# rowanz/merlot

Measured on NVIDIA H100. Metric: frame-caption segments/sec (fwd+bwd+AdamW), higher is better.
Workload: dtype bf16

## Files before the change

merlot_b200/csrc/attention.cu:

```cuda
#include "host_common.h"
#include "ptx.cuh"

namespace mb {

constexpr int AT_M = 128;
constexpr int AT_N = 128;
constexpr int AT_D = 64;
constexpr float LOG2E = 1.4426950408889634f;
constexpr float LN2 = 0.6931471805599453f;

struct AttnDev {
  int B, S, heads, H;
  const uint8_t* valid;
  float scale;
  bf16* ctx; int ld_ctx;
  float* lse;
  float* dsum;
  float* dq_accum; int ld_dq;
  size_t dq_part_stride;
  bf16* dqkv; int ld_dqkv;
  float* colsum;
  float* colsum2;
  int colsum_split;
  int colsum_valid_q;
// ... 140 lines not shown
    mbar_wait(&bar_kv[j & 1], (uint32_t)((j >> 1) & 1));
    const uint32_t ka = smem_u32(sKV + (j & 1) * 16384), va = ka + 8192;
    float s[32];
    wgmma_fence();
#pragma unroll
    for (int k = 0; k < AT_D / 16; ++k) wgmma_m64n64_ss<0, 0>(s, desc_kmajor(qa, k), desc_kmajor(ka, k), k > 0 ? 1u : 0u);
    wgmma_commit();
    wgmma_wait<0>();
    reg_fence(s);
    const int k0 = j * FK;
#pragma unroll
    for (int i = 0; i < 2; ++i) {
      uint32_t iw[2], vw[2];
#pragma unroll
      for (int w = 0; w < 2; ++w) {
        iw[w] = range_word(k0 + 32 * w, S);
        vw[w] = (HAS_MASK && vq[i]) ? s_mask[(k0 >> 5) + w] : 0xffffffffu;
        if (HAS_MASK && pair_lo[i] >= 0) vw[w] &= pair_word(k0 + 32 * w, pair_lo[i], p.pair_P, p.pair_chunk);
      }
      float mx = -INFINITY;
#pragma unroll
      for (int jj = 0; jj < 8; ++jj) {
#pragma unroll
        for (int e = 0; e < 2; ++e) {
          const int bit = (8 * jj + 2 * (lane & 3) + e) & 31, w = jj >> 2;
          float t = s[4 * jj + 2 * i + e] * sc2[i];
          t = ((vw[w] >> bit) & 1u) ? t : MASKED_LOG2;
          t = ((iw[w] >> bit) & 1u) ? t : -INFINITY;
          s[4 * jj + 2 * i + e] = t;
          mx = fmaxf(mx, t);
        }
      }
      quad_max(mx);
      const float m_new = fmaxf(m_run[i], mx);
      const float f = ex2_approx(m_run[i] - m_new);
      m_run[i] = m_new;
      float rs = 0.f;
#pragma unroll
      for (int jj = 0; jj < 8; ++jj) {
#pragma unroll
        for (int e = 0; e < 2; ++e) {
          const float pr = ex2_approx(s[4 * jj + 2 * i + e] - m_new);
          s[4 * jj + 2 * i + e] = pr;
          rs += pr;
          o[4 * jj + 2 * i + e] *= f;
        }
      }
      l_run[i] = l_run[i] * f + rs;
    }
    if (DROP) {
#pragma unroll
      for (int x = 0; x < 32; ++x)
        if (!((zq >> x) & 1u)) s[x] = 0.f;
    }
    wgmma_fence();
#pragma unroll
    for (int kk = 0; kk < FK / 16; ++kk) {
      uint32_t a[4];
      acc_to_afrag(s, kk, a);
      wgmma_m64n64_rs<1>(o, a, desc_mnmajor(va, kk, 0), 1u);
    }
    wgmma_commit();
    wgmma_wait<0>();
    reg_fence(o);
    __syncthreads();
    if (tid == 0 && j + 2 < n_kv) load_kv(j + 2);
  }

#pragma unroll
  for (int i = 0; i < 2; ++i) {
    quad_sum(l_run[i]);
    const int q = q0 + wg * 64 + wq * 16 + (lane >> 2) + 8 * i;
    if (!q_in[i]) continue;
    const float inv = (DROP ? p.drop_scale : 1.0f) / l_run[i];
    bf16* dst = p.ctx + (size_t)(tok0 + q) * p.ld_ctx + h * AT_D + 2 * (lane & 3);
#pragma unroll
    for (int jj = 0; jj < 8; ++jj)
      *reinterpret_cast<uint32_t*>(dst + 8 * jj) = pack_bf16x2(o[4 * jj + 2 * i] * inv, o[4 * jj + 2 * i + 1] * inv);
    if ((lane & 3) == 0 && p.lse) p.lse[((size_t)b * p.heads + h) * S + q] = (m_run[i] + log2f(l_run[i])) * LN2;
  }
}

constexpr int BQ = 64;
constexpr int MAX_DQ_PARTS = 4;
constexpr int BWD_THREADS = 256;
constexpr int BWD_SMEM = 32768 + 32768 + 16384 + 1024 + 512 + 64 + 1024;

__device__ __forceinline__ uint32_t attn_keep_bits_keyrows(const AttnDev& p, uint64_t drop_bh, uint64_t drop_key, uint64_t n16, int q0,
                                                           int lane) {
  uint32_t z = 0;
#pragma unroll
  for (int jp = 0; jp < BQ / 16; ++jp) {
#pragma unroll
    for (int e = 0; e < 2; ++e) {
      const uint64_t blk = ((drop_bh + (uint64_t)((q0 >> 4) + jp)) * 8 + 2 * (lane & 3) + e) * n16 * 8 + drop_key;
      const uint4 r = attn_dropout_words(p.drop_seed, p.drop_site, blk);
      const uint32_t w[4] = {r.x, r.y, r.z, r.w};
#pragma unroll
      for (int qh = 0; qh < 2; ++qh)
#pragma unroll
        for (int i = 0; i < 2; ++i)
          z |= ((w[2 * qh + i] >> 16) >= p.drop_thresh16 ? 1u : 0u) << (4 * (2 * jp + qh) + 2 * i + e);
    }
  }
  return z;
}

template <bool HAS_MASK, bool DQ_ATOMIC, bool DROP>
__global__ void __launch_bounds__(BWD_THREADS, 1)
attn_bwd_kernel(const __grid_constant__ CUtensorMap tm_kv, const __grid_constant__ CUtensorMap tm_q,
                const __grid_constant__ CUtensorMap tm_do, const AttnDev p) {
  extern __shared__ uint8_t smem_raw[];
  uint8_t* smem = reinterpret_cast<uint8_t*>((reinterpret_cast<uintptr_t>(smem_raw) + 1023) & ~uintptr_t(1023));
  uint8_t* sK = smem;
  uint8_t* sV = smem + 16384;
  uint8_t* sQd = smem + 32768;
  uint8_t* sdST = smem + 65536;
  float* s_nlse = reinterpret_cast<float*>(smem + 81920);
  float* s_dsum = s_nlse + 2 * BQ;
  uint32_t* s_mask = reinterpret_cast<uint32_t*>(s_dsum + 2 * BQ);
  uint64_t* bars = reinterpret_cast<uint64_t*>(reinterpret_cast<uint8_t*>(s_mask) + 512);
  uint64_t *bar_kv = bars, *bar_q = bars + 1 ;

  const int tid = threadIdx.x, lane = tid & 31;
  const int warp = __shfl_sync(0xffffffffu, tid >> 5, 0);
  const int wg = warp >> 2, wq = warp & 3;
  const int kt = blockIdx.x, h = blockIdx.y, b = blockIdx.z;
  pdl_launch_dependents();
  const int S = p.S, H = p.H;
  const int k0 = kt * AT_N, tok0 = b * S;
  const int n_q = (S + BQ - 1) / BQ;

  if (tid == 0) {
    tma_prefetch_desc(&tm_kv); tma_prefetch_desc(&tm_q); tma_prefetch_desc(&tm_do);
    mbar_init(bar_kv, 1); mbar_init(&bar_q[0], 1); mbar_init(&bar_q[1], 1);
    fence_barrier_init();
  }
  __syncthreads();
  pdl_wait();
  auto load_q = [&](int c) {
    uint8_t* buf = sQd + (c & 1) * 16384;
    mbar_arrive_expect_tx(&bar_q[c & 1], 16384);
    tma_load_2d(buf, &tm_q, &bar_q[c & 1], h * AT_D, tok0 + c * BQ);
    tma_load_2d(buf + 8192, &tm_do, &bar_q[c & 1], h * AT_D, tok0 + c * BQ);
  };
  if (tid == 0) {
    mbar_arrive_expect_tx(bar_kv, 32768);
    tma_load_2d(sK, &tm_kv, bar_kv, H + h * AT_D, tok0 + k0);
    tma_load_2d(sV, &tm_kv, bar_kv, 2 * H + h * AT_D, tok0 + k0);
    load_q(0);
    if (n_q > 1) load_q(1);
  }
  const size_t st0 = ((size_t)b * p.heads + h) * S;
  auto stage_stats = [&](int c) {
    const int q = c * BQ + tid;
    s_nlse[(c & 1) * BQ + tid] = (q < S) ? -p.lse[st0 + q] * LOG2E : 0.f;
    s_dsum[(c & 1) * BQ + tid] = (q < S) ? p.dsum[st0 + q] : 0.f;
  };
  if (tid < BQ) stage_stats(0);
  if (HAS_MASK) build_mask(s_mask, p.valid + tok0, n_q * BQ, S);
  __syncthreads();

  bool k_in[2], vk[2];
  int pair_lo[2];
#pragma unroll
  for (int i = 0; i < 2; ++i) {
    const int kk = k0 + wg * 64 + wq * 16 + (lane >> 2) + 8 * i;
    k_in[i] = kk < S;
    vk[i] = k_in[i] ? (HAS_MASK ? p.valid[tok0 + kk] != 0 : true) : false;
    pair_lo[i] = HAS_MASK ? pair_lo_of(kk, p.pair_P, p.pair_chunk) : -1;
  }
  const float sc2 = p.scale * LOG2E;
  float dv[32], dk[32];
#pragma unroll
  for (int i = 0; i < 32; ++i) { dv[i] = 0.f; dk[i] = 0.f; }
  float* dq_base = p.dq_accum + (DQ_ATOMIC ? (size_t)0 : (size_t)kt * p.dq_part_stride);
  uint64_t drop_n16 = 0, drop_bh = 0, drop_key = 0;
  if (DROP) {
    drop_n16 = (uint64_t)((S + 15) >> 4);
    drop_bh = ((uint64_t)b * p.heads + h) * drop_n16;
    drop_key = (uint64_t)((k0 + wg * 64 + wq * 16) >> 4) * 8 + (lane >> 2);
  }

  mbar_wait(bar_kv, 0);
  const uint32_t ka = smem_u32(sK) + wg * 8192, va = smem_u32(sV) + wg * 8192;
  const uint32_t dsa = smem_u32(sdST);
  for (int c = 0; c < n_q; ++c) {
    const int bb = c & 1, q0 = c * BQ;
    mbar_wait(&bar_q[bb], (uint32_t)((c >> 1) & 1));
    const uint32_t qa = smem_u32(sQd + bb * 16384), da = qa + 8192;
    float s[32], dp[32];
    wgmma_fence();
#pragma unroll
    for (int k = 0; k < AT_D / 16; ++k) wgmma_m64n64_ss<0, 0>(s, desc_kmajor(ka, k), desc_kmajor(qa, k), k > 0 ? 1u : 0u);
#pragma unroll
    for (int k = 0; k < AT_D / 16; ++k) wgmma_m64n64_ss<0, 0>(dp, desc_kmajor(va, k), desc_kmajor(da, k), k > 0 ? 1u : 0u);
    wgmma_commit();
    wgmma_wait<0>();
    reg_fence(s);
    reg_fence(dp);
    const float* nlse = s_nlse + bb * BQ;
    const float* dsm = s_dsum + bb * BQ;
    uint32_t iw[2], qw[2];
#pragma unroll
    for (int w = 0; w < 2; ++w) {
      iw[w] = range_word(q0 + 32 * w, S);
      qw[w] = HAS_MASK ? s_mask[(q0 >> 5) + w] : 0xffffffffu;
    }
    const uint32_t zk = DROP ? attn_keep_bits_keyrows(p, drop_bh, drop_key, drop_n16, q0, lane) : 0u;
#pragma unroll
    for (int i = 0; i < 2; ++i) {
      uint32_t aw[2];
#pragma unroll
      for (int w = 0; w < 2; ++w)
        aw[w] = (HAS_MASK && pair_lo[i] >= 0) ? pair_word(q0 + 32 * w, pair_lo[i], p.pair_P, p.pair_chunk) : 0xffffffffu;
      const int row = wg * 64 + wq * 16 + (lane >> 2) + 8 * i;
#pragma unroll
      for (int jj = 0; jj < 8; ++jj) {
        float pv[2], dsv[2];
#pragma unroll
        for (int e = 0; e < 2; ++e) {
          const int col = 8 * jj + 2 * (lane & 3) + e, bit = col & 31, w = jj >> 2;
          float t = s[4 * jj + 2 * i + e] * sc2;
          t = (vk[i] && ((aw[w] >> bit) & 1u)) ? t : MASKED_LOG2;
          t = ((qw[w] >> bit) & 1u) ? t : 0.f;
          float pr = ex2_approx(t + nlse[col]);
          pr = (k_in[i] && ((iw[w] >> bit) & 1u)) ? pr : 0.f;
          const float gq = ((qw[w] >> bit) & 1u) ? pr : 0.f;
          if (DROP) {
            const float zs = ((zk >> (4 * jj + 2 * i + e)) & 1u) ? p.drop_scale : 0.f;
            pv[e] = pr * zs;
            dsv[e] = (dp[4 * jj + 2 * i + e] * zs - dsm[col]) * gq;
          } else {
            pv[e] = pr;
            dsv[e] = (dp[4 * jj + 2 * i + e] - dsm[col]) * gq;
          }
        }
        s[4 * jj + 2 * i] = pv[0]; s[4 * jj + 2 * i + 1] = pv[1];
        dp[4 * jj + 2 * i] = dsv[0]; dp[4 * jj + 2 * i + 1] = dsv[1];
        *reinterpret_cast<uint32_t*>(sdST + row * 128 + ((jj ^ (row & 7)) << 4) + (lane & 3) * 4) = pack_bf16x2(dsv[0], dsv[1]);
      }
    }
    wgmma_fence();
#pragma unroll
    for (int kk = 0; kk < BQ / 16; ++kk) {
      uint32_t a[4];
      acc_to_afrag(s, kk, a);
      wgmma_m64n64_rs<1>(dv, a, desc_mnmajor(da, kk, 0), 1u);
    }
#pragma unroll
    for (int kk = 0; kk < BQ / 16; ++kk) {
      uint32_t a[4];
      acc_to_afrag(dp, kk, a);
      wgmma_m64n64_rs<1>(dk, a, desc_mnmajor(qa, kk, 0), 1u);
    }
    wgmma_commit();
    fence_proxy_async_smem();
    asm volatile("bar.sync 1, 256;" ::: "memory");
    float dq[16];
    wgmma_fence();
#pragma unroll
    for (int k = 0; k < AT_N / 16; ++k)
      wgmma_m64n32_ss<1, 1>(dq, desc_mnmajor(dsa, k, 0), desc_mnmajor(smem_u32(sK) + wg * 64, k, 0), k > 0 ? 1u : 0u);
    wgmma_commit();
    wgmma_wait<0>();
    reg_fence(dv);
    reg_fence(dk);
    reg_fence(dq);
#pragma unroll
    for (int i = 0; i < 2; ++i) {
      const int q = q0 + wq * 16 + (lane >> 2) + 8 * i;
      if (q >= S) continue;
      float* dst = dq_base + (size_t)(tok0 + q) * p.ld_dq + h * AT_D + wg * 32 + 2 * (lane & 3);
#pragma unroll
      for (int jj = 0; jj < 4; ++jj) {
        const float v0 = dq[4 * jj + 2 * i], v1 = dq[4 * jj + 2 * i + 1];
        if (DQ_ATOMIC) {
          asm volatile("red.global.add.v2.f32 [%0], {%1, %2};" ::"l"(dst + 8 * jj), "f"(v0), "f"(v1) : "memory");
        } else {
          *reinterpret_cast<float2*>(dst + 8 * jj) = make_float2(v0, v1);
        }
      }
    }
    if (tid < BQ && c + 1 < n_q) stage_stats(c + 1);
    __syncthreads();
    if (tid == 0 && c + 2 < n_q) load_q(c + 2);
  }
#pragma unroll
  for (int i = 0; i < 2; ++i) {
    const int key = k0 + wg * 64 + wq * 16 + (lane >> 2) + 8 * i;
    if (key >= S) continue;
    bf16* dst = p.dqkv + (size_t)(tok0 + key) * p.ld_dqkv + h * AT_D + 2 * (lane & 3);
#pragma unroll
    for (int jj = 0; jj < 8; ++jj) {
      *reinterpret_cast<uint32_t*>(dst + H + 8 * jj) = pack_bf16x2(dk[4 * jj + 2 * i] * p.scale, dk[4 * jj + 2 * i + 1] * p.scale);
      *reinterpret_cast<uint32_t*>(dst + 2 * H + 8 * jj) = pack_bf16x2(dv[4 * jj + 2 * i], dv[4 * jj + 2 * i + 1]);
    }
  }
}

__global__ void attn_dsum_kernel(const bf16* __restrict__ o, const bf16* __restrict__ d_o, int ld, float* __restrict__ dsum,
                                 int B, int S, int heads) {
  pdl_launch_dependents();
  pdl_wait();
  const long long gid = (long long)blockIdx.x * blockDim.x + threadIdx.x;
  const long long item = gid >> 3;
  const int sub = (int)(gid & 7);
  const long long total = (long long)B * S * heads;
  float acc = 0.f;
  if (item < total) {
    const int hh = (int)(item % heads);
    const long long tok = item / heads;
    const size_t off = (size_t)tok * ld + hh * AT_D + sub * 8;
    uint4 a = __ldg(reinterpret_cast<const uint4*>(o + off));
    uint4 g = __ldg(reinterpret_cast<const uint4*>(d_o + off));
    const uint32_t* pa = reinterpret_cast<const uint32_t*>(&a);
    const uint32_t* pg = reinterpret_cast<const uint32_t*>(&g);
#pragma unroll
    for (int i = 0; i < 4; ++i) {
      float2 x = unpack_bf16x2(pa[i]), y = unpack_bf16x2(pg[i]);
      acc += x.x * y.x + x.y * y.y;
    }
  }
  acc += __shfl_xor_sync(0xffffffffu, acc, 1);
  acc += __shfl_xor_sync(0xffffffffu, acc, 2);
  acc += __shfl_xor_sync(0xffffffffu, acc, 4);
  if (item < total && sub == 0) {
    const int hh = (int)(item % heads);
    const long long tok = item / heads;
    const int bb = (int)(tok / S), q = (int)(tok % S);
    dsum[((size_t)bb * heads + hh) * S + q] = acc;
  }
}

__global__ void __launch_bounds__(256) attn_dqkv_finish_kernel(float* __restrict__ dq, int ld_dq, bf16* __restrict__ dqkv, int ld_dqkv,
                                                               long long rows, int H, float* __restrict__ bias_grad, int n_parts,
                                                               size_t part_stride, float scale) {
  __shared__ float sred[8][256];
  pdl_launch_dependents();
  pdl_wait();
  const int lane = threadIdx.x & 31, warp = threadIdx.x >> 5;
  const int col = blockIdx.x * 256 + lane * 8;
  float acc[8] = {0, 0, 0, 0, 0, 0, 0, 0};
  if (col < 3 * H) {
    for (long long r = (long long)blockIdx.y * 8 + warp; r < rows; r += (long long)gridDim.y * 8) {
      float v[8];
      bf16* o = dqkv + (size_t)r * ld_dqkv + col;
      if (col < H) {
        float4* src = reinterpret_cast<float4*>(dq + (size_t)r * ld_dq + col);
        float4 a = src[0], b = src[1];
        if (n_parts == 0) {
          src[0] = make_float4(0.f, 0.f, 0.f, 0.f);
          src[1] = make_float4(0.f, 0.f, 0.f, 0.f);
        } else {
          for (int t = 1; t < n_parts; ++t) {
            const float4* s2 = reinterpret_cast<const float4*>(dq + (size_t)t * part_stride + (size_t)r * ld_dq + col);
            const float4 c = s2[0], d = s2[1];
            a.x += c.x; a.y += c.y; a.z += c.z; a.w += c.w;
            b.x += d.x; b.y += d.y; b.z += d.z; b.w += d.w;
          }
        }
        const uint4 pk = make_uint4(pack_bf16x2(a.x * scale, a.y * scale), pack_bf16x2(a.z * scale, a.w * scale),
                                    pack_bf16x2(b.x * scale, b.y * scale), pack_bf16x2(b.z * scale, b.w * scale));
        *reinterpret_cast<uint4*>(o) = pk;
        const uint32_t* pu = reinterpret_cast<const uint32_t*>(&pk);
#pragma unroll
        for (int i = 0; i < 4; ++i) { const float2 f = unpack_bf16x2(pu[i]); v[2 * i] = f.x; v[2 * i + 1] = f.y; }
      } else {
        const uint4 u = *reinterpret_cast<const uint4*>(o);
        const uint32_t* pu = reinterpret_cast<const uint32_t*>(&u);
#pragma unroll
        for (int i = 0; i < 4; ++i) { const float2 f = unpack_bf16x2(pu[i]); v[2 * i] = f.x; v[2 * i + 1] = f.y; }
      }
#pragma unroll
      for (int i = 0; i < 8; ++i) acc[i] += v[i];
    }
  }
#pragma unroll
  for (int i = 0; i < 8; ++i) sred[warp][lane * 8 + i] = acc[i];
  __syncthreads();
  const int c = threadIdx.x;
  if (bias_grad != nullptr && blockIdx.x * 256 + c < 3 * H) {
    float s2 = 0.f;
#pragma unroll
    for (int w = 0; w < 8; ++w) s2 += sred[w][c];
    atomicAdd(bias_grad + blockIdx.x * 256 + c, s2);
  }
}

constexpr int CS_THREADS = 256;
constexpr int CS_SMEM = 16384 + 2 * 8192 + 512 + 512 + 64 + 1024;

template <bool HAS_MASK, bool DROP>
__global__ void __launch_bounds__(CS_THREADS, 2) attn_colsum_kernel(const __grid_constant__ CUtensorMap tm_k, const __grid_constant__ CUtensorMap tm_q,
                                                                    const AttnDev p) {
  extern __shared__ uint8_t smem_raw[];
  uint8_t* smem = reinterpret_cast<uint8_t*>((reinterpret_cast<uintptr_t>(smem_raw) + 1023) & ~uintptr_t(1023));
  uint8_t* sK = smem;
  uint8_t* sQ = smem + 16384;
  float* s_nlse = reinterpret_cast<float*>(smem + 32768);
  uint32_t* s_mask = reinterpret_cast<uint32_t*>(smem + 32768 + 512);
  uint64_t* bars = reinterpret_cast<uint64_t*>(smem + 32768 + 1024);
  uint64_t *bar_k = bars, *bar_q = bars + 1 ;
  const int tid = threadIdx.x, lane = tid & 31;
  const int warp = __shfl_sync(0xffffffffu, tid >> 5, 0);
  const int wg = warp >> 2, wq = warp & 3;
  const int k0 = blockIdx.x * AT_N, h = blockIdx.y, b = blockIdx.z;
  const int S = p.S, H = p.H, tok0 = b * S;
  const int n_q = (S + BQ - 1) / BQ;
  pdl_launch_dependents();
  if (tid == 0) {
    tma_prefetch_desc(&tm_k); tma_prefetch_desc(&tm_q);
    mbar_init(bar_k, 1); mbar_init(&bar_q[0], 1); mbar_init(&bar_q[1], 1);
    fence_barrier_init();
  }
  __syncthreads();
  pdl_wait();
  auto load_q = [&](int c) {
    mbar_arrive_expect_tx(&bar_q[c & 1], 8192);
    tma_load_2d(sQ + (c & 1) * 8192, &tm_q, &bar_q[c & 1], h * AT_D, tok0 + c * BQ);
  };
  if (tid == 0) {
    mbar_arrive_expect_tx(bar_k, 16384);
    tma_load_2d(sK, &tm_k, bar_k, H + h * AT_D, tok0 + k0);
    load_q(0);
    if (n_q > 1) load_q(1);
  }
  auto stage_lse = [&](int c) {
    const int q = c * BQ + tid;
    s_nlse[(c & 1) * BQ + tid] = (q < S) ? -p.lse[((size_t)b * p.heads + h) * S + q] * LOG2E : 0.f;
  };
  if (tid < BQ) stage_lse(0);
  if (HAS_MASK) build_mask(s_mask, p.valid + tok0, n_q * BQ, S);
  __syncthreads();

  bool k_in[2], vk[2];
  int pair_lo[2];
// ... 273 lines not shown
```

merlot_b200/csrc/ptx.cuh:

```cuda
#pragma once
#include <cuda.h>
#include <cuda_runtime.h>
#include <cuda_bf16.h>
#include <stdint.h>
#include <stdio.h>

namespace mb {

typedef __nv_bfloat16 bf16;

__device__ __forceinline__ uint32_t smem_u32(const void* p) {
  return static_cast<uint32_t>(__cvta_generic_to_shared(p));
}

__device__ __forceinline__ void pdl_launch_dependents() { asm volatile("griddepcontrol.launch_dependents;" ::: "memory"); }
__device__ __forceinline__ void pdl_wait() { asm volatile("griddepcontrol.wait;" ::: "memory"); }

__device__ __forceinline__ bool elect_one() {
  uint32_t pred;
  asm volatile(
      "{\n\t.reg .pred p;\n\t"
      "elect.sync _|p, 0xffffffff;\n\t"
      "selp.u32 %0, 1, 0, p;\n\t}"
      : "=r"(pred));
  return pred != 0;
}

__device__ __forceinline__ void mbar_init(uint64_t* bar, uint32_t count) {
  asm volatile("mbarrier.init.shared::cta.b64 [%0], %1;" ::"r"(smem_u32(bar)), "r"(count) : "memory");
}
__device__ __forceinline__ void fence_barrier_init() {
  asm volatile("fence.mbarrier_init.release.cluster;" ::: "memory");
}
__device__ __forceinline__ void fence_proxy_async_smem() {
  asm volatile("fence.proxy.async.shared::cta;" ::: "memory");
}
__device__ __forceinline__ void mbar_arrive_expect_tx(uint64_t* bar, uint32_t bytes) {
  asm volatile("mbarrier.arrive.expect_tx.shared::cta.b64 _, [%0], %1;" ::"r"(smem_u32(bar)), "r"(bytes)
               : "memory");
}
__device__ __forceinline__ void mbar_arrive(uint64_t* bar) {
  asm volatile("mbarrier.arrive.shared::cta.b64 _, [%0];" ::"r"(smem_u32(bar)) : "memory");
}
__device__ __forceinline__ bool mbar_try_wait(uint64_t* bar, uint32_t parity) {
  uint32_t ok;
  asm volatile(
      "{\n\t.reg .pred p;\n\t"
      "mbarrier.try_wait.parity.shared::cta.b64 p, [%1], %2;\n\t"
      "selp.u32 %0, 1, 0, p;\n\t}"
      : "=r"(ok)
      : "r"(smem_u32(bar)), "r"(parity)
      : "memory");
  return ok != 0;
}
#ifndef MB_WAIT_LIMIT_CYCLES
#define MB_WAIT_LIMIT_CYCLES (4000000000LL)
#endif
__device__ __forceinline__ void mbar_wait(uint64_t* bar, uint32_t parity) {
  if (mbar_try_wait(bar, parity)) return;
  long long t0 = clock64();
  while (!mbar_try_wait(bar, parity)) {
    if (clock64() - t0 > MB_WAIT_LIMIT_CYCLES) asm volatile("trap;");
  }
}

__device__ __forceinline__ void mbar_wait_warp(uint64_t* bar, uint32_t parity) {
  if ((threadIdx.x & 31) == 0) mbar_wait(bar, parity);
  __syncwarp();
}

__device__ __forceinline__ void tma_prefetch_desc(const CUtensorMap* m) {
  asm volatile("prefetch.tensormap [%0];" ::"l"(reinterpret_cast<uint64_t>(m)) : "memory");
}
__device__ __forceinline__ void tma_load_2d(void* smem_dst, const CUtensorMap* m, uint64_t* bar, int c0, int c1) {
  asm volatile(
      "cp.async.bulk.tensor.2d.shared::cluster.global.mbarrier::complete_tx::bytes [%0], [%1, {%3, %4}], [%2];" ::
          "r"(smem_u32(smem_dst)),
      "l"(reinterpret_cast<uint64_t>(m)), "r"(smem_u32(bar)), "r"(c0), "r"(c1)
      : "memory");
}
__device__ __forceinline__ void tma_load_3d(void* smem_dst, const CUtensorMap* m, uint64_t* bar, int c0, int c1,
                                            int c2) {
  asm volatile(
      "cp.async.bulk.tensor.3d.shared::cluster.global.mbarrier::complete_tx::bytes [%0], [%1, {%3, %4, %5}], [%2];" ::
          "r"(smem_u32(smem_dst)),
      "l"(reinterpret_cast<uint64_t>(m)), "r"(smem_u32(bar)), "r"(c0), "r"(c1), "r"(c2)
      : "memory");
}

__device__ __forceinline__ void wgmma_fence() { asm volatile("wgmma.fence.sync.aligned;" ::: "memory"); }
__device__ __forceinline__ void wgmma_commit() { asm volatile("wgmma.commit_group.sync.aligned;" ::: "memory"); }
template <int N>
__device__ __forceinline__ void wgmma_wait() { asm volatile("wgmma.wait_group.sync.aligned %0;" ::"n"(N) : "memory"); }
template <int R>
__device__ __forceinline__ void reg_fence(float (&d)[R]) {
#pragma unroll
  for (int i = 0; i < R; ++i) asm volatile("" : "+f"(d[i])::"memory");
}

template <int TA, int TB>
__device__ __forceinline__ void wgmma_m64n32_ss(float (&d)[16], uint64_t da, uint64_t db, uint32_t scale_d) {
  asm volatile(
      "{\n\t.reg .pred p;\n\t"
      "setp.ne.b32 p, %18, 0;\n\t"
      "wgmma.mma_async.sync.aligned.m64n32k16.f32.bf16.bf16 "
      "{%0, %1, %2, %3, %4, %5, %6, %7, %8, %9, %10, %11, %12, %13, %14, %15}, %16, %17, p, 1, 1, %19, %20;\n\t}"
      : "+f"(d[0]), "+f"(d[1]), "+f"(d[2]), "+f"(d[3]), "+f"(d[4]), "+f"(d[5]), "+f"(d[6]), "+f"(d[7]), "+f"(d[8]), "+f"(d[9]), "+f"(d[10]), "+f"(d[11]), "+f"(d[12]), "+f"(d[13]), "+f"(d[14]), "+f"(d[15])
      : "l"(da), "l"(db), "r"(scale_d), "n"(TA), "n"(TB));
}
template <int TA, int TB>
__device__ __forceinline__ void wgmma_m64n64_ss(float (&d)[32], uint64_t da, uint64_t db, uint32_t scale_d) {
  asm volatile(
      "{\n\t.reg .pred p;\n\t"
      "setp.ne.b32 p, %34, 0;\n\t"
      "wgmma.mma_async.sync.aligned.m64n64k16.f32.bf16.bf16 "
      "{%0, %1, %2, %3, %4, %5, %6, %7, %8, %9, %10, %11, %12, %13, %14, %15, %16, %17, %18, %19, %20, %21, %22, %23, %24, %25, %26, %27, %28, %29, %30, %31}, %32, %33, p, 1, 1, %35, %36;\n\t}"
      : "+f"(d[0]), "+f"(d[1]), "+f"(d[2]), "+f"(d[3]), "+f"(d[4]), "+f"(d[5]), "+f"(d[6]), "+f"(d[7]), "+f"(d[8]), "+f"(d[9]), "+f"(d[10]), "+f"(d[11]), "+f"(d[12]), "+f"(d[13]), "+f"(d[14]), "+f"(d[15]), "+f"(d[16]), "+f"(d[17]), "+f"(d[18]), "+f"(d[19]), "+f"(d[20]), "+f"(d[21]), "+f"(d[22]), "+f"(d[23]), "+f"(d[24]), "+f"(d[25]), "+f"(d[26]), "+f"(d[27]), "+f"(d[28]), "+f"(d[29]), "+f"(d[30]), "+f"(d[31])
      : "l"(da), "l"(db), "r"(scale_d), "n"(TA), "n"(TB));
}
template <int TA, int TB>
__device__ __forceinline__ void wgmma_m64n128_ss(float (&d)[64], uint64_t da, uint64_t db, uint32_t scale_d) {
  asm volatile(
      "{\n\t.reg .pred p;\n\t"
      "setp.ne.b32 p, %66, 0;\n\t"
      "wgmma.mma_async.sync.aligned.m64n128k16.f32.bf16.bf16 "
      "{%0, %1, %2, %3, %4, %5, %6, %7, %8, %9, %10, %11, %12, %13, %14, %15, %16, %17, %18, %19, %20, %21, %22, %23, %24, %25, %26, %27, %28, %29, %30, %31, %32, %33, %34, %35, %36, %37, %38, %39, %40, %41, %42, %43, %44, %45, %46, %47, %48, %49, %50, %51, %52, %53, %54, %55, %56, %57, %58, %59, %60, %61, %62, %63}, %64, %65, p, 1, 1, %67, %68;\n\t}"
      : "+f"(d[0]), "+f"(d[1]), "+f"(d[2]), "+f"(d[3]), "+f"(d[4]), "+f"(d[5]), "+f"(d[6]), "+f"(d[7]), "+f"(d[8]), "+f"(d[9]), "+f"(d[10]), "+f"(d[11]), "+f"(d[12]), "+f"(d[13]), "+f"(d[14]), "+f"(d[15]), "+f"(d[16]), "+f"(d[17]), "+f"(d[18]), "+f"(d[19]), "+f"(d[20]), "+f"(d[21]), "+f"(d[22]), "+f"(d[23]), "+f"(d[24]), "+f"(d[25]), "+f"(d[26]), "+f"(d[27]), "+f"(d[28]), "+f"(d[29]), "+f"(d[30]), "+f"(d[31]), "+f"(d[32]), "+f"(d[33]), "+f"(d[34]), "+f"(d[35]), "+f"(d[36]), "+f"(d[37]), "+f"(d[38]), "+f"(d[39]), "+f"(d[40]), "+f"(d[41]), "+f"(d[42]), "+f"(d[43]), "+f"(d[44]), "+f"(d[45]), "+f"(d[46]), "+f"(d[47]), "+f"(d[48]), "+f"(d[49]), "+f"(d[50]), "+f"(d[51]), "+f"(d[52]), "+f"(d[53]), "+f"(d[54]), "+f"(d[55]), "+f"(d[56]), "+f"(d[57]), "+f"(d[58]), "+f"(d[59]), "+f"(d[60]), "+f"(d[61]), "+f"(d[62]), "+f"(d[63])
      : "l"(da), "l"(db), "r"(scale_d), "n"(TA), "n"(TB));
}
template <int TA, int TB>
__device__ __forceinline__ void wgmma_m64n192_ss(float (&d)[96], uint64_t da, uint64_t db, uint32_t scale_d) {
  asm volatile(
      "{\n\t.reg .pred p;\n\t"
      "setp.ne.b32 p, %98, 0;\n\t"
      "wgmma.mma_async.sync.aligned.m64n192k16.f32.bf16.bf16 "
      "{%0, %1, %2, %3, %4, %5, %6, %7, %8, %9, %10, %11, %12, %13, %14, %15, %16, %17, %18, %19, %20, %21, %22, %23, %24, %25, %26, %27, %28, %29, %30, %31, %32, %33, %34, %35, %36, %37, %38, %39, %40, %41, %42, %43, %44, %45, %46, %47, %48, %49, %50, %51, %52, %53, %54, %55, %56, %57, %58, %59, %60, %61, %62, %63, %64, %65, %66, %67, %68, %69, %70, %71, %72, %73, %74, %75, %76, %77, %78, %79, %80, %81, %82, %83, %84, %85, %86, %87, %88, %89, %90, %91, %92, %93, %94, %95}, %96, %97, p, 1, 1, %99, %100;\n\t}"
      : "+f"(d[0]), "+f"(d[1]), "+f"(d[2]), "+f"(d[3]), "+f"(d[4]), "+f"(d[5]), "+f"(d[6]), "+f"(d[7]), "+f"(d[8]), "+f"(d[9]), "+f"(d[10]), "+f"(d[11]), "+f"(d[12]), "+f"(d[13]), "+f"(d[14]), "+f"(d[15]), "+f"(d[16]), "+f"(d[17]), "+f"(d[18]), "+f"(d[19]), "+f"(d[20]), "+f"(d[21]), "+f"(d[22]), "+f"(d[23]), "+f"(d[24]), "+f"(d[25]), "+f"(d[26]), "+f"(d[27]), "+f"(d[28]), "+f"(d[29]), "+f"(d[30]), "+f"(d[31]), "+f"(d[32]), "+f"(d[33]), "+f"(d[34]), "+f"(d[35]), "+f"(d[36]), "+f"(d[37]), "+f"(d[38]), "+f"(d[39]), "+f"(d[40]), "+f"(d[41]), "+f"(d[42]), "+f"(d[43]), "+f"(d[44]), "+f"(d[45]), "+f"(d[46]), "+f"(d[47]), "+f"(d[48]), "+f"(d[49]), "+f"(d[50]), "+f"(d[51]), "+f"(d[52]), "+f"(d[53]), "+f"(d[54]), "+f"(d[55]), "+f"(d[56]), "+f"(d[57]), "+f"(d[58]), "+f"(d[59]), "+f"(d[60]), "+f"(d[61]), "+f"(d[62]), "+f"(d[63]), "+f"(d[64]), "+f"(d[65]), "+f"(d[66]), "+f"(d[67]), "+f"(d[68]), "+f"(d[69]), "+f"(d[70]), "+f"(d[71]), "+f"(d[72]), "+f"(d[73]), "+f"(d[74]), "+f"(d[75]), "+f"(d[76]), "+f"(d[77]), "+f"(d[78]), "+f"(d[79]), "+f"(d[80]), "+f"(d[81]), "+f"(d[82]), "+f"(d[83]), "+f"(d[84]), "+f"(d[85]), "+f"(d[86]), "+f"(d[87]), "+f"(d[88]), "+f"(d[89]), "+f"(d[90]), "+f"(d[91]), "+f"(d[92]), "+f"(d[93]), "+f"(d[94]), "+f"(d[95])
      : "l"(da), "l"(db), "r"(scale_d), "n"(TA), "n"(TB));
}
template <int TA, int TB>
__device__ __forceinline__ void wgmma_m64n256_ss(float (&d)[128], uint64_t da, uint64_t db, uint32_t scale_d) {
  asm volatile(
      "{\n\t.reg .pred p;\n\t"
      "setp.ne.b32 p, %130, 0;\n\t"
      "wgmma.mma_async.sync.aligned.m64n256k16.f32.bf16.bf16 "
      "{%0, %1, %2, %3, %4, %5, %6, %7, %8, %9, %10, %11, %12, %13, %14, %15, %16, %17, %18, %19, %20, %21, %22, %23, %24, %25, %26, %27, %28, %29, %30, %31, %32, %33, %34, %35, %36, %37, %38, %39, %40, %41, %42, %43, %44, %45, %46, %47, %48, %49, %50, %51, %52, %53, %54, %55, %56, %57, %58, %59, %60, %61, %62, %63, %64, %65, %66, %67, %68, %69, %70, %71, %72, %73, %74, %75, %76, %77, %78, %79, %80, %81, %82, %83, %84, %85, %86, %87, %88, %89, %90, %91, %92, %93, %94, %95, %96, %97, %98, %99, %100, %101, %102, %103, %104, %105, %106, %107, %108, %109, %110, %111, %112, %113, %114, %115, %116, %117, %118, %119, %120, %121, %122, %123, %124, %125, %126, %127}, %128, %129, p, 1, 1, %131, %132;\n\t}"
      : "+f"(d[0]), "+f"(d[1]), "+f"(d[2]), "+f"(d[3]), "+f"(d[4]), "+f"(d[5]), "+f"(d[6]), "+f"(d[7]), "+f"(d[8]), "+f"(d[9]), "+f"(d[10]), "+f"(d[11]), "+f"(d[12]), "+f"(d[13]), "+f"(d[14]), "+f"(d[15]), "+f"(d[16]), "+f"(d[17]), "+f"(d[18]), "+f"(d[19]), "+f"(d[20]), "+f"(d[21]), "+f"(d[22]), "+f"(d[23]), "+f"(d[24]), "+f"(d[25]), "+f"(d[26]), "+f"(d[27]), "+f"(d[28]), "+f"(d[29]), "+f"(d[30]), "+f"(d[31]), "+f"(d[32]), "+f"(d[33]), "+f"(d[34]), "+f"(d[35]), "+f"(d[36]), "+f"(d[37]), "+f"(d[38]), "+f"(d[39]), "+f"(d[40]), "+f"(d[41]), "+f"(d[42]), "+f"(d[43]), "+f"(d[44]), "+f"(d[45]), "+f"(d[46]), "+f"(d[47]), "+f"(d[48]), "+f"(d[49]), "+f"(d[50]), "+f"(d[51]), "+f"(d[52]), "+f"(d[53]), "+f"(d[54]), "+f"(d[55]), "+f"(d[56]), "+f"(d[57]), "+f"(d[58]), "+f"(d[59]), "+f"(d[60]), "+f"(d[61]), "+f"(d[62]), "+f"(d[63]), "+f"(d[64]), "+f"(d[65]), "+f"(d[66]), "+f"(d[67]), "+f"(d[68]), "+f"(d[69]), "+f"(d[70]), "+f"(d[71]), "+f"(d[72]), "+f"(d[73]), "+f"(d[74]), "+f"(d[75]), "+f"(d[76]), "+f"(d[77]), "+f"(d[78]), "+f"(d[79]), "+f"(d[80]), "+f"(d[81]), "+f"(d[82]), "+f"(d[83]), "+f"(d[84]), "+f"(d[85]), "+f"(d[86]), "+f"(d[87]), "+f"(d[88]), "+f"(d[89]), "+f"(d[90]), "+f"(d[91]), "+f"(d[92]), "+f"(d[93]), "+f"(d[94]), "+f"(d[95]), "+f"(d[96]), "+f"(d[97]), "+f"(d[98]), "+f"(d[99]), "+f"(d[100]), "+f"(d[101]), "+f"(d[102]), "+f"(d[103]), "+f"(d[104]), "+f"(d[105]), "+f"(d[106]), "+f"(d[107]), "+f"(d[108]), "+f"(d[109]), "+f"(d[110]), "+f"(d[111]), "+f"(d[112]), "+f"(d[113]), "+f"(d[114]), "+f"(d[115]), "+f"(d[116]), "+f"(d[117]), "+f"(d[118]), "+f"(d[119]), "+f"(d[120]), "+f"(d[121]), "+f"(d[122]), "+f"(d[123]), "+f"(d[124]), "+f"(d[125]), "+f"(d[126]), "+f"(d[127])
      : "l"(da), "l"(db), "r"(scale_d), "n"(TA), "n"(TB));
}
template <int TB>
__device__ __forceinline__ void wgmma_m64n64_rs(float (&d)[32], const uint32_t (&a)[4], uint64_t db, uint32_t scale_d) {
  asm volatile(
      "{\n\t.reg .pred p;\n\t"
      "setp.ne.b32 p, %37, 0;\n\t"
      "wgmma.mma_async.sync.aligned.m64n64k16.f32.bf16.bf16 "
      "{%0, %1, %2, %3, %4, %5, %6, %7, %8, %9, %10, %11, %12, %13, %14, %15, %16, %17, %18, %19, %20, %21, %22, %23, %24, %25, %26, %27, %28, %29, %30, %31}, {%32, %33, %34, %35}, %36, p, 1, 1, %38;\n\t}"
      : "+f"(d[0]), "+f"(d[1]), "+f"(d[2]), "+f"(d[3]), "+f"(d[4]), "+f"(d[5]), "+f"(d[6]), "+f"(d[7]), "+f"(d[8]), "+f"(d[9]), "+f"(d[10]), "+f"(d[11]), "+f"(d[12]), "+f"(d[13]), "+f"(d[14]), "+f"(d[15]), "+f"(d[16]), "+f"(d[17]), "+f"(d[18]), "+f"(d[19]), "+f"(d[20]), "+f"(d[21]), "+f"(d[22]), "+f"(d[23]), "+f"(d[24]), "+f"(d[25]), "+f"(d[26]), "+f"(d[27]), "+f"(d[28]), "+f"(d[29]), "+f"(d[30]), "+f"(d[31])
      : "r"(a[0]), "r"(a[1]), "r"(a[2]), "r"(a[3]), "l"(db), "r"(scale_d), "n"(TB));
}

__device__ __forceinline__ uint64_t make_smem_desc_sw128(uint32_t smem_addr, uint32_t lbo_bytes, uint32_t sbo_bytes) {
  uint64_t d = 0;
  d |= (uint64_t)((smem_addr & 0x3FFFF) >> 4);
  d |= (uint64_t)((lbo_bytes >> 4) & 0x3FFF) << 16;
  d |= (uint64_t)((sbo_bytes >> 4) & 0x3FFF) << 32;
  d |= (uint64_t)1 << 62;
  return d;
}
__device__ __forceinline__ uint64_t desc_kmajor(uint32_t tile_addr, int k16) {
  return make_smem_desc_sw128(tile_addr + 32u * k16, 0, 1024);
}
__device__ __forceinline__ uint64_t desc_mnmajor(uint32_t tile_addr, int k16, uint32_t chunk_bytes) {
  return make_smem_desc_sw128(tile_addr + 2048u * k16, chunk_bytes, 1024);
}

__device__ __forceinline__ uint32_t sw128_offset(uint32_t row, uint32_t chunk16) {
  return row * 128u + ((chunk16 ^ (row & 7u)) << 4);
}

__device__ __forceinline__ float gelu_erf(float x) { return x * 0.5f * (1.0f + erff(x * 0.70710678118654752440f)); }
__device__ __forceinline__ float gelu_erf_grad(float x) {
  float cdf = 0.5f * (1.0f + erff(x * 0.70710678118654752440f));
  float pdf = 0.39894228040143267794f * __expf(-0.5f * x * x);
  return cdf + x * pdf;
}
__device__ __forceinline__ float ex2_approx(float x) {
  float y;
  asm("ex2.approx.ftz.f32 %0, %1;" : "=f"(y) : "f"(x));
  return y;
}
__device__ __forceinline__ float rcp_approx(float x) {
  float y;
  asm("rcp.approx.ftz.f32 %0, %1;" : "=f"(y) : "f"(x));
  return y;
}
__device__ __forceinline__ float normal_cdf_fast(float x, float* e_out) {
  const float t = rcp_approx(fmaf(0.23164190f, fabsf(x), 1.0f));
  const float e = ex2_approx((x * x) * -0.72134752f);
  float poly = fmaf(t, 0.5307027145f, -0.7265760135f);
  poly = fmaf(poly, t, 0.7107068705f);
  poly = fmaf(poly, t, -0.142248368f);
  poly = fmaf(poly, t, 0.127414796f);
  const float half_erfc = (poly * t) * e;
  if (e_out) *e_out = e;
  return x >= 0.f ? 1.0f - half_erfc : half_erfc;
}
__device__ __forceinline__ float gelu_erf_fast(float x) { return x * normal_cdf_fast(x, nullptr); }
__device__ __forceinline__ float gelu_erf_grad_fast(float x) {
  float e;
  const float cdf = normal_cdf_fast(x, &e);
  return fmaf(x * 0.39894228040143267794f, e, cdf);
}
__device__ __forceinline__ uint32_t pack_bf16x2(float lo, float hi) {
  __nv_bfloat162 v = __floats2bfloat162_rn(lo, hi);
  return *reinterpret_cast<uint32_t*>(&v);
}
__device__ __forceinline__ float2 unpack_bf16x2(uint32_t u) {
  __nv_bfloat162 v = *reinterpret_cast<__nv_bfloat162*>(&u);
  return __bfloat1622float2(v);
}

__device__ __forceinline__ uint4 philox4x32_7(uint4 ctr, uint2 key) {
  const uint32_t M0 = 0xD2511F53u, M1 = 0xCD9E8D57u, W0 = 0x9E3779B9u, W1 = 0xBB67AE85u;
#pragma unroll
  for (int i = 0; i < 7; ++i) {
    uint32_t hi0 = __umulhi(M0, ctr.x), lo0 = M0 * ctr.x;
    uint32_t hi1 = __umulhi(M1, ctr.z), lo1 = M1 * ctr.z;
    ctr = make_uint4(hi1 ^ ctr.y ^ key.x, lo1, hi0 ^ ctr.w ^ key.y, lo0);
    key.x += W0;
    key.y += W1;
  }
  return ctr;
}
__device__ __forceinline__ uint32_t dropout_keep8(uint64_t seed, uint32_t site, uint64_t idx8, uint32_t thresh16) {
  uint4 r = philox4x32_7(make_uint4((uint32_t)idx8, (uint32_t)(idx8 >> 32), site, 0x4d45524cu),
                         make_uint2((uint32_t)seed, (uint32_t)(seed >> 32)));
  uint32_t w[4] = {r.x, r.y, r.z, r.w};
  uint32_t m = 0;
#pragma unroll
  for (int i = 0; i < 4; ++i) {
    m |= ((w[i] & 0xFFFFu) >= thresh16 ? 1u : 0u) << (2 * i);
// ... 12 lines not shown
```

Baseline: 1159.

## Prefetch softmax stats with cp.async and skip idle warpgroup on short key tiles

The per-query LSE and dsum stats used to be loaded synchronously at the end of each chunk. They are now issued as cp.async copies at the start of the chunk and finished, with the LSE scaled by -log2e, after the dQ work, so the global-load latency overlaps with compute. Separately, when the second warpgroup's 64 keys lie entirely past the sequence end, that warpgroup skips the S/dP GEMMs, the softmax-gradient math and the dV/dK GEMMs. Its half of the dS^T tile is zeroed once up front so the shared dQ GEMM still reads valid data. This adds an extra async-copy wait and a divergent branch inside the loop.

```diff
diff --git a/merlot_b200/csrc/attention.cu b/merlot_b200/csrc/attention.cu
--- a/merlot_b200/csrc/attention.cu
+++ b/merlot_b200/csrc/attention.cu
@@ -316,12 +316,20 @@
     if (n_q > 1) load_q(1);
   }
   const size_t st0 = ((size_t)b * p.heads + h) * S;
-  auto stage_stats = [&](int c) {
+  auto load_stats = [&](int c) {
     const int q = c * BQ + tid;
-    s_nlse[(c & 1) * BQ + tid] = (q < S) ? -p.lse[st0 + q] * LOG2E : 0.f;
-    s_dsum[(c & 1) * BQ + tid] = (q < S) ? p.dsum[st0 + q] : 0.f;
+    const uint32_t n = q < S ? 4u : 0u;
+    cp_async_4(&s_nlse[(c & 1) * BQ + tid], p.lse + st0 + (q < S ? q : 0), n);
+    cp_async_4(&s_dsum[(c & 1) * BQ + tid], p.dsum + st0 + (q < S ? q : 0), n);
   };
-  if (tid < BQ) stage_stats(0);
+  auto finish_stats = [&](int c) {
+    cp_async_wait_all();
+    s_nlse[(c & 1) * BQ + tid] = -s_nlse[(c & 1) * BQ + tid] * LOG2E;
+  };
+  if (tid < BQ) {
+    load_stats(0);
+    finish_stats(0);
+  }
   if (HAS_MASK) build_mask(s_mask, p.valid + tok0, n_q * BQ, S);
   __syncthreads();
 
@@ -346,79 +354,86 @@
     drop_key = (uint64_t)((k0 + wg * 64 + wq * 16) >> 4) * 8 + (lane >> 2);
   }
 
+  const bool idle = wg == 1 && S - k0 <= 64;
+  if (idle) {
+    for (int x = tid - 128; x < 64 * 128 / 16; x += 128) reinterpret_cast<uint4*>(sdST + 64 * 128)[x] = make_uint4(0, 0, 0, 0);
+  }
   mbar_wait(bar_kv, 0);
   const uint32_t ka = smem_u32(sK) + wg * 8192, va = smem_u32(sV) + wg * 8192;
   const uint32_t dsa = smem_u32(sdST);
   for (int c = 0; c < n_q; ++c) {
     const int bb = c & 1, q0 = c * BQ;
+    if (tid < BQ && c + 1 < n_q) load_stats(c + 1);
     mbar_wait(&bar_q[bb], (uint32_t)((c >> 1) & 1));
     const uint32_t qa = smem_u32(sQd + bb * 16384), da = qa + 8192;
-    float s[32], dp[32];
-    wgmma_fence();
-#pragma unroll
-    for (int k = 0; k < AT_D / 16; ++k) wgmma_m64n64_ss<0, 0>(s, desc_kmajor(ka, k), desc_kmajor(qa, k), k > 0 ? 1u : 0u);
-#pragma unroll
-    for (int k = 0; k < AT_D / 16; ++k) wgmma_m64n64_ss<0, 0>(dp, desc_kmajor(va, k), desc_kmajor(da, k), k > 0 ? 1u : 0u);
-    wgmma_commit();
-    wgmma_wait<0>();
-    reg_fence(s);
-    reg_fence(dp);
-    const float* nlse = s_nlse + bb * BQ;
-    const float* dsm = s_dsum + bb * BQ;
-    uint32_t iw[2], qw[2];
-#pragma unroll
-    for (int w = 0; w < 2; ++w) {
-      iw[w] = range_word(q0 + 32 * w, S);
-      qw[w] = HAS_MASK ? s_mask[(q0 >> 5) + w] : 0xffffffffu;
-    }
-    const uint32_t zk = DROP ? attn_keep_bits_keyrows(p, drop_bh, drop_key, drop_n16, q0, lane) : 0u;
-#pragma unroll
-    for (int i = 0; i < 2; ++i) {
-      uint32_t aw[2];
-#pragma unroll
-      for (int w = 0; w < 2; ++w)
-        aw[w] = (HAS_MASK && pair_lo[i] >= 0) ? pair_word(q0 + 32 * w, pair_lo[i], p.pair_P, p.pair_chunk) : 0xffffffffu;
-      const int row = wg * 64 + wq * 16 + (lane >> 2) + 8 * i;
-#pragma unroll
-      for (int jj = 0; jj < 8; ++jj) {
-        float pv[2], dsv[2];
-#pragma unroll
-        for (int e = 0; e < 2; ++e) {
-          const int col = 8 * jj + 2 * (lane & 3) + e, bit = col & 31, w = jj >> 2;
-          float t = s[4 * jj + 2 * i + e] * sc2;
-          t = (vk[i] && ((aw[w] >> bit) & 1u)) ? t : MASKED_LOG2;
-          t = ((qw[w] >> bit) & 1u) ? t : 0.f;
-          float pr = ex2_approx(t + nlse[col]);
-          pr = (k_in[i] && ((iw[w] >> bit) & 1u)) ? pr : 0.f;
-          const float gq = ((qw[w] >> bit) & 1u) ? pr : 0.f;
-          if (DROP) {
-            const float zs = ((zk >> (4 * jj + 2 * i + e)) & 1u) ? p.drop_scale : 0.f;
-            pv[e] = pr * zs;
-            dsv[e] = (dp[4 * jj + 2 * i + e] * zs - dsm[col]) * gq;
-          } else {
-            pv[e] = pr;
-            dsv[e] = (dp[4 * jj + 2 * i + e] - dsm[col]) * gq;
+    if (!idle) {
+      float s[32], dp[32];
+      wgmma_fence();
+#pragma unroll
+      for (int k = 0; k < AT_D / 16; ++k) wgmma_m64n64_ss<0, 0>(s, desc_kmajor(ka, k), desc_kmajor(qa, k), k > 0 ? 1u : 0u);
+#pragma unroll
+      for (int k = 0; k < AT_D / 16; ++k) wgmma_m64n64_ss<0, 0>(dp, desc_kmajor(va, k), desc_kmajor(da, k), k > 0 ? 1u : 0u);
+      wgmma_commit();
+      wgmma_wait<0>();
+      reg_fence(s);
+      reg_fence(dp);
+      const float* nlse = s_nlse + bb * BQ;
+      const float* dsm = s_dsum + bb * BQ;
+      uint32_t iw[2], qw[2];
+#pragma unroll
+      for (int w = 0; w < 2; ++w) {
+        iw[w] = range_word(q0 + 32 * w, S);
+        qw[w] = HAS_MASK ? s_mask[(q0 >> 5) + w] : 0xffffffffu;
+      }
+      const uint32_t zk = DROP ? attn_keep_bits_keyrows(p, drop_bh, drop_key, drop_n16, q0, lane) : 0u;
+#pragma unroll
+      for (int i = 0; i < 2; ++i) {
+        uint32_t aw[2];
+#pragma unroll
+        for (int w = 0; w < 2; ++w)
+          aw[w] = (HAS_MASK && pair_lo[i] >= 0) ? pair_word(q0 + 32 * w, pair_lo[i], p.pair_P, p.pair_chunk) : 0xffffffffu;
+        const int row = wg * 64 + wq * 16 + (lane >> 2) + 8 * i;
+#pragma unroll
+        for (int jj = 0; jj < 8; ++jj) {
+          float pv[2], dsv[2];
+#pragma unroll
+          for (int e = 0; e < 2; ++e) {
+            const int col = 8 * jj + 2 * (lane & 3) + e, bit = col & 31, w = jj >> 2;
+            float t = s[4 * jj + 2 * i + e] * sc2;
+            t = (vk[i] && ((aw[w] >> bit) & 1u)) ? t : MASKED_LOG2;
+            t = ((qw[w] >> bit) & 1u) ? t : 0.f;
+            float pr = ex2_approx(t + nlse[col]);
+            pr = (k_in[i] && ((iw[w] >> bit) & 1u)) ? pr : 0.f;
+            const float gq = ((qw[w] >> bit) & 1u) ? pr : 0.f;
+            if (DROP) {
+              const float zs = ((zk >> (4 * jj + 2 * i + e)) & 1u) ? p.drop_scale : 0.f;
+              pv[e] = pr * zs;
+              dsv[e] = (dp[4 * jj + 2 * i + e] * zs - dsm[col]) * gq;
+            } else {
+              pv[e] = pr;
+              dsv[e] = (dp[4 * jj + 2 * i + e] - dsm[col]) * gq;
+            }
           }
+          s[4 * jj + 2 * i] = pv[0]; s[4 * jj + 2 * i + 1] = pv[1];
+          dp[4 * jj + 2 * i] = dsv[0]; dp[4 * jj + 2 * i + 1] = dsv[1];
+          *reinterpret_cast<uint32_t*>(sdST + row * 128 + ((jj ^ (row & 7)) << 4) + (lane & 3) * 4) = pack_bf16x2(dsv[0], dsv[1]);
         }
-        s[4 * jj + 2 * i] = pv[0]; s[4 * jj + 2 * i + 1] = pv[1];
-        dp[4 * jj + 2 * i] = dsv[0]; dp[4 * jj + 2 * i + 1] = dsv[1];
-        *reinterpret_cast<uint32_t*>(sdST + row * 128 + ((jj ^ (row & 7)) << 4) + (lane & 3) * 4) = pack_bf16x2(dsv[0], dsv[1]);
-      }
-    }
-    wgmma_fence();
-#pragma unroll
-    for (int kk = 0; kk < BQ / 16; ++kk) {
-      uint32_t a[4];
-      acc_to_afrag(s, kk, a);
-      wgmma_m64n64_rs<1>(dv, a, desc_mnmajor(da, kk, 0), 1u);
-    }
-#pragma unroll
-    for (int kk = 0; kk < BQ / 16; ++kk) {
-      uint32_t a[4];
-      acc_to_afrag(dp, kk, a);
-      wgmma_m64n64_rs<1>(dk, a, desc_mnmajor(qa, kk, 0), 1u);
-    }
-    wgmma_commit();
+      }
+      wgmma_fence();
+#pragma unroll
+      for (int kk = 0; kk < BQ / 16; ++kk) {
+        uint32_t a[4];
+        acc_to_afrag(s, kk, a);
+        wgmma_m64n64_rs<1>(dv, a, desc_mnmajor(da, kk, 0), 1u);
+      }
+#pragma unroll
+      for (int kk = 0; kk < BQ / 16; ++kk) {
+        uint32_t a[4];
+        acc_to_afrag(dp, kk, a);
+        wgmma_m64n64_rs<1>(dk, a, desc_mnmajor(qa, kk, 0), 1u);
+      }
+      wgmma_commit();
+    }
     fence_proxy_async_smem();
     asm volatile("bar.sync 1, 256;" ::: "memory");
     float dq[16];
@@ -446,7 +461,7 @@
         }
       }
     }
-    if (tid < BQ && c + 1 < n_q) stage_stats(c + 1);
+    if (tid < BQ && c + 1 < n_q) finish_stats(c + 1);
     __syncthreads();
     if (tid == 0 && c + 2 < n_q) load_q(c + 2);
   }
diff --git a/merlot_b200/csrc/ptx.cuh b/merlot_b200/csrc/ptx.cuh
--- a/merlot_b200/csrc/ptx.cuh
+++ b/merlot_b200/csrc/ptx.cuh
@@ -87,6 +87,13 @@
       "l"(reinterpret_cast<uint64_t>(m)), "r"(smem_u32(bar)), "r"(c0), "r"(c1), "r"(c2)
       : "memory");
 }
+
+__device__ __forceinline__ void cp_async_4(void* smem_dst, const void* gsrc, uint32_t src_bytes) {
+  asm volatile("cp.async.ca.shared.global [%0], [%1], 4, %2;" ::"r"(smem_u32(smem_dst)), "l"(reinterpret_cast<uint64_t>(gsrc)),
+               "r"(src_bytes)
+               : "memory");
+}
+__device__ __forceinline__ void cp_async_wait_all() { asm volatile("cp.async.wait_all;" ::: "memory"); }
 
 __device__ __forceinline__ void wgmma_fence() { asm volatile("wgmma.fence.sync.aligned;" ::: "memory"); }
 __device__ __forceinline__ void wgmma_commit() { asm volatile("wgmma.commit_group.sync.aligned;" ::: "memory"); }
```

Measured after the change: 1182, median of 6. +2.0%, better.
